# underdoc-wang/MPGCN

Measured on NVIDIA H100. Metric: OD-cells/sec (B*T*N^2), MPGCN hot path fwd+bwd, higher is better.
Workload: dtype f16

## Files before the change

mpgcn_b200/csrc/common.cuh:

```cuda
#pragma once

#include <cuda.h>
#include <cuda_fp16.h>
#include <cuda_runtime.h>
#include <stdint.h>
#include <stdio.h>

#if defined(__CUDA_ARCH__) && !defined(__CUDA_ARCH_FEAT_SM90_ALL)
#error "mpgcn_b200 must be compiled for sm_90a (-gencode arch=compute_90a,code=sm_90a)"
#endif

namespace mpgcn {

void set_error(const char* fmt, ...);
#define MPGCN_CHECK(cond, ...)                                                     \
  do {                                                                             \
    if (!(cond)) {                                                                 \
      ::mpgcn::set_error(__VA_ARGS__);                                             \
      return 1;                                                                    \
    }                                                                              \
  } while (0)
#define MPGCN_CUDA(call)                                                           \
  do {                                                                             \
    cudaError_t e__ = (call);                                                      \
// ... 7 lines not shown

#ifdef __CUDACC__
__device__ __forceinline__ uint32_t smem_u32(const void* p) {
  return static_cast<uint32_t>(__cvta_generic_to_shared(p));
}

__device__ __forceinline__ void mbar_init(uint64_t* bar, uint32_t count) {
  asm volatile("mbarrier.init.shared::cta.b64 [%0], %1;" ::"r"(smem_u32(bar)), "r"(count) : "memory");
}
__device__ __forceinline__ void fence_barrier_init() {
  asm volatile("fence.mbarrier_init.release.cluster;" ::: "memory");
}
__device__ __forceinline__ void fence_proxy_async_smem() {
  asm volatile("fence.proxy.async.shared::cta;" ::: "memory");
}
__device__ __forceinline__ void mbar_arrive_expect_tx(uint64_t* bar, uint32_t bytes) {
  asm volatile("mbarrier.arrive.expect_tx.shared::cta.b64 _, [%0], %1;" ::"r"(smem_u32(bar)), "r"(bytes) : "memory");
}
__device__ __forceinline__ void mbar_arrive(uint64_t* bar) {
  asm volatile("mbarrier.arrive.shared::cta.b64 _, [%0];" ::"r"(smem_u32(bar)) : "memory");
}
__device__ __forceinline__ bool mbar_try_wait(uint64_t* bar, uint32_t parity) {
  uint32_t ok;
  asm volatile(
      "{\n\t.reg .pred p;\n\t"
      "mbarrier.try_wait.parity.shared::cta.b64 p, [%1], %2;\n\t"
      "selp.u32 %0, 1, 0, p;\n\t}"
      : "=r"(ok)
      : "r"(smem_u32(bar)), "r"(parity)
      : "memory");
  return ok != 0;
}
static __device__ __noinline__ void mbar_wait_slow(uint64_t* bar, uint32_t parity) {
  const long long t0 = clock64();
  uint32_t spins = 0;
  while (!mbar_try_wait(bar, parity)) {
    if (((++spins) & 0xFFFu) == 0 && (clock64() - t0) > 6000000000LL) {
      printf("mpgcn_b200: mbarrier wait timed out (block %d thread %d)\n", blockIdx.x, threadIdx.x);
      __trap();
    }
  }
}
__device__ __forceinline__ void mbar_wait(uint64_t* bar, uint32_t parity) {
  if (mbar_try_wait(bar, parity)) return;
  mbar_wait_slow(bar, parity);
}
__device__ __forceinline__ void mbar_wait_inline(uint64_t* bar, uint32_t parity) {
  if (mbar_try_wait(bar, parity)) return;
  const long long t0 = clock64();
  while (!mbar_try_wait(bar, parity))
    if (clock64() - t0 > 6000000000LL) __trap();
}

__device__ __forceinline__ void tma_prefetch_desc(const CUtensorMap* map) {
  asm volatile("prefetch.tensormap [%0];" ::"l"(map) : "memory");
}
__device__ __forceinline__ void tma_load_4d(void* smem_dst, const CUtensorMap* map, uint64_t* bar,
                                            int c0, int c1, int c2, int c3) {
  asm volatile(
      "cp.async.bulk.tensor.4d.shared::cluster.global.mbarrier::complete_tx::bytes"
      " [%0], [%1, {%3, %4, %5, %6}], [%2];"
      ::"r"(smem_u32(smem_dst)), "l"(map), "r"(smem_u32(bar)), "r"(c0), "r"(c1), "r"(c2), "r"(c3)
      : "memory");
}

__device__ __forceinline__ void wgmma_fence() { asm volatile("wgmma.fence.sync.aligned;" ::: "memory"); }
__device__ __forceinline__ void wgmma_commit() { asm volatile("wgmma.commit_group.sync.aligned;" ::: "memory"); }
template <int N>
__device__ __forceinline__ void wgmma_wait() { asm volatile("wgmma.wait_group.sync.aligned %0;" ::"n"(N) : "memory"); }
__device__ __forceinline__ void named_bar_sync(int id, int count) { asm volatile("bar.sync %0, %1;" ::"r"(id), "r"(count) : "memory"); }

constexpr uint32_t GMMA_SW128 = 1u, GMMA_SW64 = 2u;
__device__ __forceinline__ uint64_t gmma_desc_hi(uint32_t sbo_bytes, uint32_t swizzle) {
  return (static_cast<uint64_t>((sbo_bytes >> 4) & 0x3FFFu) | (static_cast<uint64_t>(swizzle) << 30)) << 32;
}
__device__ __forceinline__ uint64_t gmma_desc(uint64_t hi, uint32_t smem_addr, uint32_t lbo_bytes) {
  return hi | static_cast<uint64_t>((smem_addr >> 4) & 0x3FFFu) | (static_cast<uint64_t>((lbo_bytes >> 4) & 0x3FFFu) << 16);
}

__device__ __forceinline__ void mma_16816(float (&d)[4], const uint32_t (&a)[4], uint32_t b0, uint32_t b1) {
  asm volatile("mma.sync.aligned.m16n8k16.row.col.f32.f16.f16.f32 {%0, %1, %2, %3}, {%4, %5, %6, %7}, {%8, %9}, {%0, %1, %2, %3};"
               : "+f"(d[0]), "+f"(d[1]), "+f"(d[2]), "+f"(d[3])
               : "r"(a[0]), "r"(a[1]), "r"(a[2]), "r"(a[3]), "r"(b0), "r"(b1));
}
__device__ __forceinline__ void ldmatrix_x4(uint32_t addr, uint32_t& r0, uint32_t& r1, uint32_t& r2, uint32_t& r3) {
  asm volatile("ldmatrix.sync.aligned.m8n8.x4.shared.b16 {%0, %1, %2, %3}, [%4];" : "=r"(r0), "=r"(r1), "=r"(r2), "=r"(r3) : "r"(addr));
}
__device__ __forceinline__ void ldmatrix_x4_trans(uint32_t addr, uint32_t& r0, uint32_t& r1, uint32_t& r2, uint32_t& r3) {
  asm volatile("ldmatrix.sync.aligned.m8n8.x4.trans.shared.b16 {%0, %1, %2, %3}, [%4];" : "=r"(r0), "=r"(r1), "=r"(r2), "=r"(r3) : "r"(addr));
}

__device__ __forceinline__ __half f2h_sat(float x) { return __float2half_rn(fabsf(x) > 65504.f ? copysignf(65504.f, x) : x); }
__device__ __forceinline__ uint32_t f2h2_sat_bits(float a, float b) {
  uint32_t r;
  asm("cvt.rn.satfinite.f16x2.f32 %0, %1, %2;" : "=r"(r) : "f"(b), "f"(a));
  return r;
}
#endif

enum TmapSwizzle { TMAP_SW64 = 0, TMAP_SW128 = 1 };
int make_tmap_f16(CUtensorMap* out, const void* gptr, int rank, const uint64_t* dims, const uint64_t* strides_bytes,
                  const uint32_t* box, TmapSwizzle swz);

int device_sm_count();

struct DynSmemAttr { int bytes[64]; };
int ensure_dyn_smem_impl(const void* kernel, int bytes, DynSmemAttr& cache);
template <class Kernel>
inline int ensure_dyn_smem(Kernel kernel, int bytes, DynSmemAttr& cache) {
  return ensure_dyn_smem_impl(reinterpret_cast<const void*>(kernel), bytes, cache);
}

enum ProfTag {
  PROF_FWD_A = 0, PROF_FWD_MIX, PROF_FWD_B, PROF_BWD_V, PROF_BWD_DW, PROF_BWD_MIX, PROF_BWD_DX,
  PROF_SIMT_GEMM, PROF_ELEMENTWISE, PROF_LSTM_FWD, PROF_LSTM_BWD,
  PROF_LAYER_FWD, PROF_LAYER_BWD, PROF_HEAD,
  PROF_EXCHANGE,
  PROF_NUM_TAGS
};
constexpr int PROF_FIRST_REGION_TAG = PROF_LAYER_FWD;
void prof_set_next(int tag, double flops);
void prof_take_next(int* tag, double* flops);
void prof_count(int tag);
void prof_begin(int tag, double flops, cudaStream_t s);
void prof_end(cudaStream_t s);
struct ProfRegion {
  void* a = nullptr;
  int tag;
  cudaStream_t s;
  ProfRegion(int tag, double flops, cudaStream_t s);
  ~ProfRegion();
};

}
```

mpgcn_b200/csrc/lstm_tc.cu:

```cuda
#include "kernels.h"

namespace mpgcn {
namespace lstm_tc {

template <int CH>
struct Dims {
  static constexpr int CG = CH == 1 ? 8 : CH == 3 ? 4 : 3;
  static constexpr int CELLS = 16 * CG;
  static constexpr int H = 32 * CH;
  static constexpr int G4 = 4 * H;
  static constexpr int KX = H + 16;
  static constexpr int WX_LD = KX + 8;
  static constexpr int HX_LD = KX + 8;
  static constexpr int H_LD = H + 8;
  static constexpr int DA_LD = G4 + 8;
  static constexpr int NW = CG * CH;
  static constexpr int THREADS = 32 * NW;
  static constexpr int FWD_CTAS_PER_SM = CH == 1 ? 2 : 1;
  static constexpr int BWD_CTAS_PER_SM = 1;
  static constexpr int TILE_HALVES = CELLS * H * 2;
};

constexpr int WT_LD = 136;
constexpr float kLn2 = 0.69314718055994531f;
// ... 11 lines not shown
__device__ __forceinline__ uint32_t pack2(float a, float b) {
  __half2 h = __floats2half2_rn(a, b);
  return *reinterpret_cast<uint32_t*>(&h);
}
__device__ __forceinline__ uint4 pack8(const float* v) {
  return make_uint4(pack2(v[0], v[1]), pack2(v[2], v[3]), pack2(v[4], v[5]), pack2(v[6], v[7]));
}
__device__ __forceinline__ void unpack8(const uint4& v, float* f) {
  const __half2* h2 = reinterpret_cast<const __half2*>(&v);
#pragma unroll
  for (int e = 0; e < 4; ++e) {
    const float2 t = __half22float2(h2[e]);
    f[2 * e] = t.x;
    f[2 * e + 1] = t.y;
  }
}

template <int CH>
__device__ __forceinline__ int gate_row(int r) { return (r & 127) / 32 * (32 * CH) + 32 * (r >> 7) + (r & 31); }
__device__ __forceinline__ float row_scale(int r) { return ((r & 127) >> 5) == 2 ? -2.8853900817779268f : -1.4426950408889634f; }

template <int CH>
__device__ void load_wx(__half* sWx, const float* w_ih, const float* w_hh, const float* b_ih, const float* b_hh) {
  using D = Dims<CH>;
  constexpr int NCH = D::KX / 8;
  for (int e = threadIdx.x; e < D::G4 * NCH; e += blockDim.x) {
    const int r = e / NCH, ch = e % NCH, j = gate_row<CH>(r);
    const float sc = row_scale(r);
    float v[8] = {0.f, 0.f, 0.f, 0.f, 0.f, 0.f, 0.f, 0.f};
    if (ch < D::H / 8) {
#pragma unroll
      for (int i = 0; i < 8; ++i) v[i] = sc * w_hh[(size_t)j * D::H + ch * 8 + i];
    } else if (ch == D::H / 8) {
      const float wi = sc * w_ih[j], bb = sc * (b_ih[j] + b_hh[j]);
      const float wi_hi = __half2float(__float2half_rn(wi)), b_hi = __half2float(__float2half_rn(bb));
      v[0] = wi_hi; v[1] = b_hi; v[2] = wi_hi; v[3] = wi - wi_hi; v[4] = bb - b_hi;
    }
    *reinterpret_cast<uint4*>(sWx + r * D::WX_LD + ch * 8) = pack8(v);
  }
}

__device__ __forceinline__ uint32_t x_cols(float x, int q) {
  const float x_hi = x_split_hi(x);
  return q == 0 ? pack2(x_hi, 1.f) : q == 1 ? pack2(x_split_lo(x, x_hi), x_hi) : q == 2 ? pack2(1.f, 0.f) : 0u;
}

template <int CH, class AH>
__device__ __forceinline__ void gate_mma(float (&acc)[16][4], AH&& a_h, const uint32_t (&xw)[2], uint32_t wx_addr) {
  using D = Dims<CH>;
  const int lane = threadIdx.x & 31, mi = lane >> 3;
#pragma unroll
  for (int nt = 0; nt < 16; ++nt) acc[nt][0] = acc[nt][1] = acc[nt][2] = acc[nt][3] = 0.f;
#pragma unroll
  for (int kb = 0; kb <= 2 * CH; ++kb) {
    uint32_t a[4];
    if (kb < 2 * CH) a_h(kb, a);
    else { a[0] = xw[0]; a[1] = xw[1]; a[2] = 0u; a[3] = 0u; }
#pragma unroll
    for (int pr = 0; pr < 8; ++pr) {
      uint32_t b0, b1, b2, b3;
      ldmatrix_x4(wx_addr + (uint32_t)(((16 * pr + 8 * (mi >> 1) + (lane & 7)) * D::WX_LD + 16 * kb + 8 * (mi & 1)) * 2), b0, b1, b2, b3);
      mma_16816(acc[2 * pr], a, b0, b1);
      mma_16816(acc[2 * pr + 1], a, b2, b3);
    }
  }
}

__device__ __forceinline__ void cell_update(const float (&acc)[16][4], float (&c)[2][8], float (&hv)[2][8]) {
#pragma unroll
  for (int h = 0; h < 2; ++h) {
#pragma unroll
    for (int s = 0; s < 8; ++s) {
      const int jn = s >> 1, k = 2 * h + (s & 1);
      const float ai = 1.f + ex2_(fminf(acc[jn][k], 40.f));
      const float af = 1.f + ex2_(fminf(acc[4 + jn][k], 40.f));
      const float ag = 1.f + ex2_(fminf(acc[8 + jn][k], 40.f));
      const float p = 1.f + ex2_(fminf(acc[12 + jn][k], 40.f));
      const float pig = ai * ag;
      const float r = rcp_(pig * af);
      const float gi = r * (ag * af);
      const float gg = fmaf(r + r, ai * af, -1.f);
      const float gf = r * pig;
      c[h][s] = fmaf(gf, c[h][s], gi * gg);
      const float ac = 1.f + ex2_(fminf(-2.8853900817779268f * c[h][s], 40.f));
      const float r2 = rcp_(p * ac);
      hv[h][s] = (r2 * ac) * fmaf(r2 + r2, p, -1.f);
    }
  }
}

template <int CH>
__device__ __forceinline__ float cell_grad(const float (&acc)[16][4], int h, const uint4& vc, const uint4& vcp, const float (&dh)[8],
                                           float (&dc)[8], const float* s_wih, int js, int q, float (&d)[4][8]) {
  constexpr int H = Dims<CH>::H;
  float fc[8], fcp[8];
  unpack8(vc, fc);
  unpack8(vcp, fcp);
  float dx = 0.f;
#pragma unroll
  for (int s = 0; s < 8; ++s) {
    const int jn = s >> 1, k = 2 * h + (s & 1);
    const float ai = 1.f + ex2_(fminf(acc[jn][k], 40.f));
    const float af = 1.f + ex2_(fminf(acc[4 + jn][k], 40.f));
    const float ag = 1.f + ex2_(fminf(acc[8 + jn][k], 40.f));
    const float ao = 1.f + ex2_(fminf(acc[12 + jn][k], 40.f));
    const float ac = 1.f + ex2_(fminf(-2.8853900817779268f * fc[s], 40.f));
    const float pig = ai * ag;
    const float r1 = rcp_(pig * af), r2 = rcp_(ao * ac);
    const float gi = r1 * (ag * af), gg = fmaf(r1 + r1, ai * af, -1.f), gf = r1 * pig;
    const float go = r2 * ac, tcv = fmaf(r2 + r2, ao, -1.f);
    const float dhv = dh[s];
    const float dcv = fmaf(dhv * go, fmaf(-tcv, tcv, 1.f), dc[s]);
    d[3][s] = (dhv * tcv) * fmaf(-go, go, go);
    d[0][s] = (dcv * gg) * fmaf(-gi, gi, gi);
    d[1][s] = (dcv * fcp[s]) * fmaf(-gf, gf, gf);
    d[2][s] = (dcv * gi) * fmaf(-gg, gg, 1.f);
    dc[s] = dcv * gf;
    const int u = 32 * js + 8 * jn + 2 * q + (s & 1);
    dx += d[0][s] * s_wih[u] + d[1][s] * s_wih[H + u] + d[2][s] * s_wih[2 * H + u] + d[3][s] * s_wih[3 * H + u];
  }
  return dx;
}

template <int CH>
__device__ __forceinline__ size_t save_off(long long tile, int T, int t, int warp, int kind, int lane) {
  return ((size_t)tile * T + t) * Dims<CH>::TILE_HALVES + (size_t)warp * 1024 + (size_t)kind * 512 + (size_t)lane * 16;
}

template <bool SAVE>
__global__ void __launch_bounds__(Dims<1>::THREADS, Dims<1>::FWD_CTAS_PER_SM)
lstm_fwd_tc_kernel(const float* __restrict__ x_seq, const float* __restrict__ w_ih, const float* __restrict__ w_hh,
                   const float* __restrict__ b_ih, const float* __restrict__ b_hh, float* __restrict__ hT, __half* __restrict__ saved,
                   long long cells, int T, long long NN) {
  using D = Dims<1>;
  __shared__ __align__(16) __half sWx[D::G4 * D::WX_LD];
  load_wx<1>(sWx, w_ih, w_hh, b_ih, b_hh);
  __syncthreads();
  const int warp = threadIdx.x >> 5, lane = threadIdx.x & 31, g = lane >> 2, q = lane & 3;
  const uint32_t wx_addr = smem_u32(sWx);
  const long long tiles = (cells + D::CELLS - 1) / D::CELLS;
  for (long long tile = blockIdx.x; tile < tiles; tile += gridDim.x) {
    long long cell[2];
    bool live[2];
    size_t xb[2];
    float xv[2];
#pragma unroll
    for (int h = 0; h < 2; ++h) {
      cell[h] = tile * D::CELLS + warp * 16 + g + 8 * h;
      live[h] = cell[h] < cells;
      xb[h] = live[h] ? x_base(cell[h], T, NN) : 0;
      xv[h] = live[h] ? x_seq[xb[h]] : 0.f;
    }
    float c[2][8], hv[2][8];
#pragma unroll
    for (int h = 0; h < 2; ++h)
#pragma unroll
      for (int s = 0; s < 8; ++s) { c[h][s] = 0.f; hv[h][s] = 0.f; }
    for (int t = 0; t < T; ++t) {
      uint32_t hw[8], xw[2];
#pragma unroll
      for (int h = 0; h < 2; ++h) {
#pragma unroll
        for (int jn = 0; jn < 4; ++jn) hw[4 * h + jn] = pack2(hv[h][2 * jn], hv[h][2 * jn + 1]);
        xw[h] = x_cols(xv[h], q);
      }
      float acc[16][4];
      gate_mma<1>(acc, [&](int kb, uint32_t (&a)[4]) {
        a[0] = hw[2 * kb]; a[1] = hw[4 + 2 * kb]; a[2] = hw[2 * kb + 1]; a[3] = hw[4 + 2 * kb + 1];
      }, xw, wx_addr);
#pragma unroll
      for (int h = 0; h < 2; ++h) xv[h] = (live[h] && t + 1 < T) ? x_seq[xb[h] + (size_t)(t + 1) * NN] : 0.f;
      cell_update(acc, c, hv);
      if (SAVE) {
        uint4* dc = reinterpret_cast<uint4*>(saved + save_off<1>(tile, T, t, warp, 0, lane));
        uint4* dh = reinterpret_cast<uint4*>(saved + save_off<1>(tile, T, t, warp, 1, lane));
        dc[0] = pack8(c[0]); dc[1] = pack8(c[1]);
        dh[0] = pack8(hv[0]); dh[1] = pack8(hv[1]);
      }
    }
    if (hT != nullptr) {
#pragma unroll
      for (int h = 0; h < 2; ++h)
        if (live[h]) {
#pragma unroll
          for (int jn = 0; jn < 4; ++jn)
            *reinterpret_cast<float2*>(hT + (size_t)cell[h] * D::H + 8 * jn + 2 * q) = make_float2(hv[h][2 * jn], hv[h][2 * jn + 1]);
        }
    }
  }
}

constexpr size_t kBwdSavedSmem = (size_t)(Dims<1>::G4 * Dims<1>::WX_LD + Dims<1>::H * WT_LD + 2 * Dims<1>::CELLS * Dims<1>::DA_LD +
                                          2 * Dims<1>::CELLS * Dims<1>::HX_LD) * sizeof(__half) + Dims<1>::G4 * sizeof(float);

__global__ void __launch_bounds__(Dims<1>::THREADS, Dims<1>::BWD_CTAS_PER_SM)
lstm_bwd_saved_tc_kernel(const float* __restrict__ x_seq, const float* __restrict__ w_ih, const float* __restrict__ w_hh,
                         const float* __restrict__ b_ih, const float* __restrict__ b_hh, const float* __restrict__ d_hT,
                         float* __restrict__ d_w_ih, float* __restrict__ d_w_hh, float* __restrict__ d_b, float* __restrict__ d_x,
                         const __half* __restrict__ saved, const float* __restrict__ scale2, long long cells, int T, long long NN) {
  using D = Dims<1>;
  constexpr int C = D::H, CELLS = D::CELLS;
  extern __shared__ __align__(16) uint8_t smem_raw[];
  __half* sWx = reinterpret_cast<__half*>(smem_raw);
  __half* sWT = sWx + D::G4 * D::WX_LD;
  __half* sDA = sWT + C * WT_LD;
  __half* sHX = sDA + 2 * CELLS * D::DA_LD;
  float* s_wih = reinterpret_cast<float*>(sHX + 2 * CELLS * D::HX_LD);

  load_wx<1>(sWx, w_ih, w_hh, b_ih, b_hh);
  for (int e = threadIdx.x; e < D::G4 * C; e += blockDim.x) {
    const int j = e / C, u = e % C;
    sWT[u * WT_LD + j] = __float2half_rn(w_hh[e]);
  }
  for (int j = threadIdx.x; j < D::G4; j += blockDim.x) s_wih[j] = w_ih[j];
  for (int e = threadIdx.x; e < 2 * CELLS; e += blockDim.x)
    *reinterpret_cast<uint4*>(sHX + e * D::HX_LD + 40) = make_uint4(0u, 0u, 0u, 0u);
  __syncthreads();

  const int warp = threadIdx.x >> 5, lane = threadIdx.x & 31, g = lane >> 2, q = lane & 3, mi = lane >> 3;
  const uint32_t wx_addr = smem_u32(sWx), wt_addr = smem_u32(sWT), da_addr = smem_u32(sDA), hx_addr = smem_u32(sHX);
  const long long tiles = (cells + CELLS - 1) / CELLS;
  const float S = scale2[0], invS = scale2[1];
  float dw[6][4];
#pragma unroll
  for (int nt = 0; nt < 6; ++nt) dw[nt][0] = dw[nt][1] = dw[nt][2] = dw[nt][3] = 0.f;
  int step = 0;

  for (long long tile = blockIdx.x; tile < tiles; tile += gridDim.x) {
    long long cell[2];
    bool live[2];
    size_t xb[2];
    float dh[2][8], dc[2][8];
#pragma unroll
    for (int h = 0; h < 2; ++h) {
      cell[h] = tile * CELLS + warp * 16 + g + 8 * h;
      live[h] = cell[h] < cells;
      xb[h] = live[h] ? x_base(cell[h], T, NN) : 0;
#pragma unroll
      for (int s = 0; s < 8; ++s) {
        dh[h][s] = live[h] ? d_hT[(size_t)cell[h] * C + 8 * (s >> 1) + 2 * q + (s & 1)] * S : 0.f;
        dc[h][s] = 0.f;
      }
    }
    for (int t = T - 1; t >= 0; --t, ++step) {
      uint4 vc[2], vcp[2], vhp[2];
      {
        const uint4* pc = reinterpret_cast<const uint4*>(saved + save_off<1>(tile, T, t, warp, 0, lane));
        vc[0] = pc[0]; vc[1] = pc[1];
        if (t > 0) {
          const uint4* pcp = reinterpret_cast<const uint4*>(saved + save_off<1>(tile, T, t - 1, warp, 0, lane));
          const uint4* php = reinterpret_cast<const uint4*>(saved + save_off<1>(tile, T, t - 1, warp, 1, lane));
          vcp[0] = pcp[0]; vcp[1] = pcp[1]; vhp[0] = php[0]; vhp[1] = php[1];
        } else {
          vcp[0] = vcp[1] = vhp[0] = vhp[1] = make_uint4(0u, 0u, 0u, 0u);
        }
      }
      const uint32_t hw[8] = {vhp[0].x, vhp[0].y, vhp[0].z, vhp[0].w, vhp[1].x, vhp[1].y, vhp[1].z, vhp[1].w};
      float xt[2];
      uint32_t xw[2];
#pragma unroll
      for (int h = 0; h < 2; ++h) {
        xt[h] = live[h] ? x_seq[xb[h] + (size_t)t * NN] : 0.f;
        xw[h] = x_cols(xt[h], q);
      }
      float acc[16][4];
      gate_mma<1>(acc, [&](int kb, uint32_t (&a)[4]) {
        a[0] = hw[2 * kb]; a[1] = hw[4 + 2 * kb]; a[2] = hw[2 * kb + 1]; a[3] = hw[4 + 2 * kb + 1];
      }, xw, wx_addr);

      uint32_t da[16][2];
      float dx[2];
#pragma unroll
      for (int h = 0; h < 2; ++h) {
        float d[4][8];
        dx[h] = cell_grad<1>(acc, h, vc[h], vcp[h], dh[h], dc[h], s_wih, 0, q, d);
#pragma unroll
        for (int jn = 0; jn < 4; ++jn)
#pragma unroll
          for (int gt = 0; gt < 4; ++gt) da[4 * gt + jn][h] = pack2(d[gt][2 * jn], d[gt][2 * jn + 1]);
      }
      if (d_x != nullptr) {
#pragma unroll
        for (int h = 0; h < 2; ++h) {
          float v = dx[h];
          v += __shfl_xor_sync(0xffffffffu, v, 1);
          v += __shfl_xor_sync(0xffffffffu, v, 2);
          if (q == 0 && live[h]) d_x[xb[h] + (size_t)t * NN] = v * invS;
        }
      }
      if (t > 0) {
        float adh[4][4];
#pragma unroll
        for (int nt = 0; nt < 4; ++nt) adh[nt][0] = adh[nt][1] = adh[nt][2] = adh[nt][3] = 0.f;
#pragma unroll
        for (int kb = 0; kb < 8; ++kb) {
          const uint32_t a[4] = {da[2 * kb][0], da[2 * kb][1], da[2 * kb + 1][0], da[2 * kb + 1][1]};
#pragma unroll
          for (int pr = 0; pr < 2; ++pr) {
            uint32_t b0, b1, b2, b3;
            ldmatrix_x4(wt_addr + (uint32_t)(((16 * pr + 8 * (mi >> 1) + (lane & 7)) * WT_LD + 16 * kb + 8 * (mi & 1)) * 2), b0, b1, b2, b3);
            mma_16816(adh[2 * pr], a, b0, b1);
            mma_16816(adh[2 * pr + 1], a, b2, b3);
          }
        }
#pragma unroll
        for (int h = 0; h < 2; ++h)
#pragma unroll
          for (int s = 0; s < 8; ++s) dh[h][s] = adh[s >> 1][2 * h + (s & 1)];
      }
      const int buf = step & 1;
      __half* sda = sDA + buf * CELLS * D::DA_LD;
      __half* shx = sHX + buf * CELLS * D::HX_LD;
#pragma unroll
      for (int h = 0; h < 2; ++h) {
        const int row = warp * 16 + g + 8 * h;
#pragma unroll
        for (int nt = 0; nt < 16; ++nt) *reinterpret_cast<uint32_t*>(sda + row * D::DA_LD + 8 * nt + 2 * q) = da[nt][h];
#pragma unroll
        for (int jn = 0; jn < 4; ++jn) *reinterpret_cast<uint32_t*>(shx + row * D::HX_LD + 8 * jn + 2 * q) = hw[4 * h + jn];
        *reinterpret_cast<uint32_t*>(shx + row * D::HX_LD + 32 + 2 * q) = xw[h];
      }
      __syncthreads();
      const uint32_t da_b = da_addr + (uint32_t)(buf * CELLS * D::DA_LD * 2), hx_b = hx_addr + (uint32_t)(buf * CELLS * D::HX_LD * 2);
#pragma unroll
      for (int kc = 0; kc < 8; ++kc) {
        uint32_t a[4];
        ldmatrix_x4_trans(da_b + (uint32_t)(((16 * kc + 8 * (mi >> 1) + (lane & 7)) * D::DA_LD + 16 * warp + 8 * (mi & 1)) * 2), a[0], a[1], a[2], a[3]);
#pragma unroll
        for (int pr = 0; pr < 3; ++pr) {
          uint32_t b0, b1, b2, b3;
          ldmatrix_x4_trans(hx_b + (uint32_t)(((16 * kc + 8 * (mi & 1) + (lane & 7)) * D::HX_LD + 16 * pr + 8 * (mi >> 1)) * 2), b0, b1, b2, b3);
          mma_16816(dw[2 * pr], a, b0, b1);
          mma_16816(dw[2 * pr + 1], a, b2, b3);
        }
      }
    }
  }
#pragma unroll
  for (int nt = 0; nt < 5; ++nt)
#pragma unroll
    for (int i = 0; i < 4; ++i) {
      const int j = 16 * warp + g + 8 * (i >> 1), col = 8 * nt + 2 * q + (i & 1);
      const float v = dw[nt][i] * invS;
      if (col < C) atomicAdd(&d_w_hh[j * C + col], v);
      else if (col == 32 || col == 34) atomicAdd(&d_w_ih[j], v);
      else if (col == 33) atomicAdd(&d_b[j], v);
    }
}


template <int CH>
constexpr size_t kFwdWideSmem = (size_t)(Dims<CH>::G4 * Dims<CH>::WX_LD + 2 * Dims<CH>::CELLS * Dims<CH>::H_LD) * sizeof(__half);

template <int CH, bool SAVE>
__global__ void __launch_bounds__(Dims<CH>::THREADS, Dims<CH>::FWD_CTAS_PER_SM)
lstm_fwd_tcw_kernel(const float* __restrict__ x_seq, const float* __restrict__ w_ih, const float* __restrict__ w_hh,
                    const float* __restrict__ b_ih, const float* __restrict__ b_hh, float* __restrict__ hT, __half* __restrict__ saved,
                    long long cells, int T, long long NN) {
  using D = Dims<CH>;
  constexpr int CELLS = D::CELLS;
  extern __shared__ __align__(16) uint8_t smem_raw[];
  __half* sWx = reinterpret_cast<__half*>(smem_raw);
  __half* sH = sWx + D::G4 * D::WX_LD;
  load_wx<CH>(sWx, w_ih, w_hh, b_ih, b_hh);
  __syncthreads();
  const int warp = threadIdx.x >> 5, lane = threadIdx.x & 31, g = lane >> 2, q = lane & 3;
  const int cg = warp / CH, js = warp % CH;
  const uint32_t wx_addr = smem_u32(sWx + js * 128 * D::WX_LD);
  const uint32_t h_addr = smem_u32(sH + (cg * 16 + (lane & 15)) * D::H_LD + 8 * (lane >> 4));
  const long long tiles = (cells + CELLS - 1) / CELLS;
  for (long long tile = blockIdx.x; tile < tiles; tile += gridDim.x) {
    long long cell[2];
    bool live[2];
    size_t xb[2];
    float xv[2];
#pragma unroll
    for (int h = 0; h < 2; ++h) {
      cell[h] = tile * CELLS + cg * 16 + g + 8 * h;
      live[h] = cell[h] < cells;
      xb[h] = live[h] ? x_base(cell[h], T, NN) : 0;
      xv[h] = live[h] ? x_seq[xb[h]] : 0.f;
    }
    float c[2][8];
#pragma unroll
    for (int h = 0; h < 2; ++h)
#pragma unroll
      for (int s = 0; s < 8; ++s) c[h][s] = 0.f;
    for (int t = 0; t < T; ++t) {
      uint32_t xw[2];
#pragma unroll
// ... 62 lines not shown
  const uint32_t da_addr = smem_u32(sDA + (cg * 16 + (lane & 15)) * D::DA_LD + 8 * (lane >> 4));
  const long long tiles = (cells + CELLS - 1) / CELLS;
  const float S = scale2[0], invS = scale2[1];

  for (long long tile = blockIdx.x; tile < tiles; tile += gridDim.x) {
    long long cell[2];
    bool live[2];
    size_t xb[2];
    float dh[2][8], dc[2][8];
#pragma unroll
    for (int h = 0; h < 2; ++h) {
      cell[h] = tile * CELLS + cg * 16 + g + 8 * h;
      live[h] = cell[h] < cells;
      xb[h] = live[h] ? x_base(cell[h], T, NN) : 0;
#pragma unroll
      for (int s = 0; s < 8; ++s) {
        dh[h][s] = live[h] ? d_hT[(size_t)cell[h] * D::H + 32 * js + 8 * (s >> 1) + 2 * q + (s & 1)] * S : 0.f;
        dc[h][s] = 0.f;
      }
    }
    const long long dx_cell = tile * CELLS + cg * 16 + (lane & 15);
    const bool dx_live = d_x != nullptr && js == 0 && lane < 16 && dx_cell < cells;
    const size_t dx_base = dx_live ? x_base(dx_cell, T, NN) : 0;

    for (int t = T - 1; t >= 0; --t) {
      uint32_t xw[2];
#pragma unroll
      for (int h = 0; h < 2; ++h) xw[h] = x_cols(live[h] ? x_seq[xb[h] + (size_t)t * NN] : 0.f, q);
      const __half* hp = saved + (t > 0 ? save_off<CH>(tile, T, t - 1, cg * CH, 1, lane) : 0);
      float acc[16][4];
      gate_mma<CH>(acc, [&](int kb, uint32_t (&a)[4]) {
        if (t == 0) { a[0] = a[1] = a[2] = a[3] = 0u; return; }
        const uint2* p = reinterpret_cast<const uint2*>(hp + (kb >> 1) * 1024);
        const uint2 r0 = __ldg(p + (kb & 1)), r1 = __ldg(p + 2 + (kb & 1));
        a[0] = r0.x; a[1] = r1.x; a[2] = r0.y; a[3] = r1.y;
      }, xw, wx_addr);

      uint4 vc[2], vcp[2];
      {
        const uint4* pc = reinterpret_cast<const uint4*>(saved + save_off<CH>(tile, T, t, warp, 0, lane));
        vc[0] = pc[0]; vc[1] = pc[1];
        if (t > 0) {
          const uint4* pcp = reinterpret_cast<const uint4*>(saved + save_off<CH>(tile, T, t - 1, warp, 0, lane));
          vcp[0] = pcp[0]; vcp[1] = pcp[1];
        } else {
          vcp[0] = vcp[1] = make_uint4(0u, 0u, 0u, 0u);
        }
      }
      uint32_t da[16][2];
      float dx[2];
#pragma unroll
      for (int h = 0; h < 2; ++h) {
        float d[4][8];
        dx[h] = cell_grad<CH>(acc, h, vc[h], vcp[h], dh[h], dc[h], s_wih, js, q, d);
#pragma unroll
        for (int jn = 0; jn < 4; ++jn)
#pragma unroll
          for (int gt = 0; gt < 4; ++gt) {
            const float inv_s = gt == 2 ? -0.5f * kLn2 : -kLn2;
            da[4 * gt + jn][h] = pack2(inv_s * d[gt][2 * jn], inv_s * d[gt][2 * jn + 1]);
          }
        dx[h] += __shfl_xor_sync(0xffffffffu, dx[h], 1);
        dx[h] += __shfl_xor_sync(0xffffffffu, dx[h], 2);
      }
      named_bar_sync(1 + cg, 32 * CH);
#pragma unroll
      for (int h = 0; h < 2; ++h) {
        const int row = cg * 16 + g + 8 * h;
#pragma unroll
        for (int nt = 0; nt < 16; ++nt) *reinterpret_cast<uint32_t*>(sDA + row * D::DA_LD + 128 * js + 8 * nt + 2 * q) = da[nt][h];
        if (q == 0) sDX[row * CH + js] = dx[h];
      }
      named_bar_sync(1 + cg, 32 * CH);
      if (dx_live) {
        float v = 0.f;
#pragma unroll
        for (int sl = 0; sl < CH; ++sl) v += sDX[(cg * 16 + lane) * CH + sl];
        d_x[dx_base + (size_t)t * NN] = v * invS;
      }
      {
        __half* rec = da_rec + (((size_t)tile * T + t) * CELLS + cg * 16) * D::G4 + 128 * js;
#pragma unroll
        for (int i = 0; i < 8; ++i) {
          const int idx = 32 * i + lane, row = idx >> 4, ch = idx & 15;
          *reinterpret_cast<uint4*>(rec + (size_t)row * D::G4 + 8 * ch) =
              *reinterpret_cast<const uint4*>(sDA + (cg * 16 + row) * D::DA_LD + 128 * js + 8 * ch);
        }
      }
      if (t > 0) {
        float adh[4][4];
#pragma unroll
        for (int nt = 0; nt < 4; ++nt) adh[nt][0] = adh[nt][1] = adh[nt][2] = adh[nt][3] = 0.f;
#pragma unroll 4
        for (int kb = 0; kb < D::G4 / 16; ++kb) {
          uint32_t a[4];
          ldmatrix_x4(da_addr + 32 * kb, a[0], a[1], a[2], a[3]);
#pragma unroll
          for (int pr = 0; pr < 2; ++pr) {
            uint32_t b0, b1, b2, b3;
            ldmatrix_x4_trans(wx_all + (uint32_t)(((16 * kb + 8 * (mi & 1) + (lane & 7)) * D::WX_LD + 32 * js + 16 * pr + 8 * (mi >> 1)) * 2),
                              b0, b1, b2, b3);
            mma_16816(adh[2 * pr], a, b0, b1);
            mma_16816(adh[2 * pr + 1], a, b2, b3);
          }
        }
#pragma unroll
        for (int h = 0; h < 2; ++h)
// ... 90 lines not shown
using lstm_tc::Dims;

bool lstm_tc_supported(int T, int C) { return (C == 32 || C == 96 || C == 128) && T >= 1 && T <= 256; }

template <int CH>
static int lstm_grid(long long cells, int ctas_per_sm) {
  const long long tiles = (cells + Dims<CH>::CELLS - 1) / Dims<CH>::CELLS;
  long long g = (long long)ctas_per_sm * device_sm_count();
  return (int)(g < tiles ? g : tiles);
}

static long long lstm_tc_padded_cells(int B, long long NN, int C) {
  const long long tc = C == 32 ? Dims<1>::CELLS : C == 96 ? Dims<3>::CELLS : Dims<4>::CELLS;
  return ((long long)B * NN + tc - 1) / tc * tc;
}

size_t lstm_tc_saved_bytes(int B, int T, long long NN, int C) {
  return (size_t)lstm_tc_padded_cells(B, NN, C) * T * 2 * C * sizeof(__half);
}

static size_t lstm_tcw_da_bytes(int B, int T, long long NN, int C) {
  return (size_t)lstm_tc_padded_cells(B, NN, C) * T * 4 * C * sizeof(__half);
}

static size_t lstm_tc_bwd_saved_workspace_bytes(int B, int T, long long NN, int C) {
  return 1024 + (C == 32 ? 0 : align_up(lstm_tcw_da_bytes(B, T, NN, C), 256));
}

size_t lstm_tc_bwd_workspace_bytes(int B, int T, long long NN, int C) {
  return lstm_tc_bwd_saved_workspace_bytes(B, T, NN, C) + align_up(lstm_tc_saved_bytes(B, T, NN, C), 256);
}

template <int CH>
static int lstm_forward_tcw(const float* x_seq, const float* w_ih, const float* w_hh, const float* b_ih, const float* b_hh, float* hT,
                            void* saved, long long cells, int T, long long NN, cudaStream_t st) {
  using D = Dims<CH>;
  auto kern = saved ? lstm_tc::lstm_fwd_tcw_kernel<CH, true> : lstm_tc::lstm_fwd_tcw_kernel<CH, false>;
  constexpr size_t smem = lstm_tc::kFwdWideSmem<CH>;
  static DynSmemAttr attr_t = {}, attr_f = {};
  if (int e = ensure_dyn_smem(kern, (int)smem, saved ? attr_t : attr_f)) return e;
  prof_begin(PROF_LSTM_FWD, 8.0 * D::H * (D::H + 1) * (double)cells * T, st);
  kern<<<lstm_grid<CH>(cells, D::FWD_CTAS_PER_SM), D::THREADS, smem, st>>>(x_seq, w_ih, w_hh, b_ih, b_hh, hT,
                                                                           static_cast<__half*>(saved), cells, T, NN);
  prof_end(st);
  MPGCN_CUDA(cudaGetLastError());
  return 0;
}

static int lstm_backward_h32(const float* x_seq, const float* w_ih, const float* w_hh, const float* b_ih, const float* b_hh,
                             const float* d_hT, float* d_w_ih, float* d_w_hh, float* d_b, float* d_x, const void* saved,
                             void* , const float* scale2, long long cells, int T, long long NN, cudaStream_t st) {
  using D = Dims<1>;
  if (d_x) MPGCN_CUDA(cudaMemsetAsync(d_x, 0, sizeof(float) * (size_t)cells * T, st));
  static DynSmemAttr attr_b = {};
  if (int e = ensure_dyn_smem(lstm_tc::lstm_bwd_saved_tc_kernel, (int)lstm_tc::kBwdSavedSmem, attr_b)) return e;
  prof_begin(PROF_LSTM_BWD, 12.0 * D::H * (D::H + 1) * (double)cells * T, st);
  lstm_tc::lstm_bwd_saved_tc_kernel<<<lstm_grid<1>(cells, D::BWD_CTAS_PER_SM), D::THREADS, lstm_tc::kBwdSavedSmem, st>>>(
      x_seq, w_ih, w_hh, b_ih, b_hh, d_hT, d_w_ih, d_w_hh, d_b, d_x, static_cast<const __half*>(saved), scale2, cells, T, NN);
  prof_end(st);
  MPGCN_CUDA(cudaGetLastError());
  return 0;
}

template <int CH>
static int lstm_backward_tcw(const float* x_seq, const float* w_ih, const float* w_hh, const float* b_ih, const float* b_hh,
                             const float* d_hT, float* d_w_ih, float* d_w_hh, float* d_b, float* d_x, const void* saved, void* da_rec,
                             const float* scale2, long long cells, int T, long long NN, cudaStream_t st) {
  using D = Dims<CH>;
  constexpr size_t smem = lstm_tc::kWalkSmem<CH>;
  static DynSmemAttr attr_b = {};
  if (int e = ensure_dyn_smem(lstm_tc::lstm_bwd_walk_tcw_kernel<CH>, (int)smem, attr_b)) return e;
  prof_begin(PROF_LSTM_BWD, 8.0 * D::H * (D::H + 1) * (double)cells * T, st);
  lstm_tc::lstm_bwd_walk_tcw_kernel<CH><<<lstm_grid<CH>(cells, D::BWD_CTAS_PER_SM), D::THREADS, smem, st>>>(
      x_seq, w_ih, w_hh, b_ih, b_hh, d_hT, d_x, static_cast<const __half*>(saved), static_cast<__half*>(da_rec), scale2, cells, T, NN);
  prof_end(st);
  MPGCN_CUDA(cudaGetLastError());
  const long long records = (cells + D::CELLS - 1) / D::CELLS * T;
  long long splits = 4LL * device_sm_count() / CH;
  if (splits > records) splits = records;
  prof_begin(PROF_LSTM_BWD, 4.0 * D::H * (D::H + 1) * (double)cells * T, st);
  lstm_tc::lstm_dw_tcw_kernel<CH><<<dim3(CH, (unsigned)splits), lstm_tc::DW_THREADS, 0, st>>>(
      x_seq, static_cast<const __half*>(saved), static_cast<const __half*>(da_rec), d_w_ih, d_w_hh, d_b, scale2, cells, T, NN);
  prof_end(st);
  MPGCN_CUDA(cudaGetLastError());
  return 0;
}

int lstm_last_forward_tc(const float* x_seq, const float* w_ih, const float* w_hh, const float* b_ih, const float* b_hh, float* hT,
                         void* saved, int B, int T, long long NN, int C, cudaStream_t st) {
  using D = Dims<1>;
  const long long cells = (long long)B * NN;
  MPGCN_CHECK(saved == nullptr || (reinterpret_cast<uintptr_t>(saved) & 15) == 0, "lstm forward: saved buffer must be 16-byte aligned");
  if (C == 96) return lstm_forward_tcw<3>(x_seq, w_ih, w_hh, b_ih, b_hh, hT, saved, cells, T, NN, st);
  if (C == 128) return lstm_forward_tcw<4>(x_seq, w_ih, w_hh, b_ih, b_hh, hT, saved, cells, T, NN, st);
  MPGCN_CHECK(C == D::H, "lstm forward: no tensor-core kernel for hidden=%d", C);
  auto kern = saved ? lstm_tc::lstm_fwd_tc_kernel<true> : lstm_tc::lstm_fwd_tc_kernel<false>;
  prof_begin(PROF_LSTM_FWD, 8.0 * C * (C + 1) * (double)cells * T, st);
  kern<<<lstm_grid<1>(cells, D::FWD_CTAS_PER_SM), D::THREADS, 0, st>>>(x_seq, w_ih, w_hh, b_ih, b_hh, hT, static_cast<__half*>(saved),
                                                                       cells, T, NN);
  prof_end(st);
  MPGCN_CUDA(cudaGetLastError());
  return 0;
}

int lstm_last_backward_tc(const float* x_seq, const float* w_ih, const float* w_hh, const float* b_ih, const float* b_hh,
                          const float* d_hT, float* d_w_ih, float* d_w_hh, float* d_b_ih, float* d_b_hh, float* d_x, const void* saved,
                          int B, int T, long long NN, int C, void* ws, size_t ws_bytes, const float* d_hT_absmax, cudaStream_t st) {
  const long long cells = (long long)B * NN;
  const size_t need = saved ? lstm_tc_bwd_saved_workspace_bytes(B, T, NN, C) : lstm_tc_bwd_workspace_bytes(B, T, NN, C);
  MPGCN_CHECK(ws != nullptr && ws_bytes >= need, "lstm backward: workspace too small (%zu < %zu)", ws_bytes, need);
// ... 26 lines not shown
```

Before: 487.8 million.

## Pipeline LSTM backward with cp.async ring and mbarrier-decoupled weight-gradient GEMM

The saved-state LSTM backward kernel now prefetches the saved c/h states and x inputs through a 3-slot cp.async ring in shared memory. The block-wide __syncthreads before the weight-gradient MMA is replaced by full/empty mbarriers, so each warp computes the dW product for the previous step while the next step proceeds. The kernel is templated on whether d_x is needed so the dx arithmetic can be compiled out. The x-column bias MMA uses a smaller m16n8k8 and the dW accumulator tile shrinks from 6 to 5 n-tiles. This costs more shared memory, which may lower occupancy, and adds barrier and ring-slot bookkeeping.

```diff
diff --git a/mpgcn_b200/csrc/common.cuh b/mpgcn_b200/csrc/common.cuh
--- a/mpgcn_b200/csrc/common.cuh
+++ b/mpgcn_b200/csrc/common.cuh
@@ -83,6 +83,16 @@
     if (clock64() - t0 > 6000000000LL) __trap();
 }
 
+__device__ __forceinline__ void cp_async16(void* smem_dst, const void* src) {
+  asm volatile("cp.async.cg.shared.global [%0], [%1], 16;" ::"r"(smem_u32(smem_dst)), "l"(src) : "memory");
+}
+__device__ __forceinline__ void cp_async4(void* smem_dst, const void* src) {
+  asm volatile("cp.async.ca.shared.global [%0], [%1], 4;" ::"r"(smem_u32(smem_dst)), "l"(src) : "memory");
+}
+__device__ __forceinline__ void cp_async_commit() { asm volatile("cp.async.commit_group;" ::: "memory"); }
+template <int N>
+__device__ __forceinline__ void cp_async_wait() { asm volatile("cp.async.wait_group %0;" ::"n"(N) : "memory"); }
+
 __device__ __forceinline__ void tma_prefetch_desc(const CUtensorMap* map) {
   asm volatile("prefetch.tensormap [%0];" ::"l"(map) : "memory");
 }
@@ -113,6 +123,17 @@
   asm volatile("mma.sync.aligned.m16n8k16.row.col.f32.f16.f16.f32 {%0, %1, %2, %3}, {%4, %5, %6, %7}, {%8, %9}, {%0, %1, %2, %3};"
                : "+f"(d[0]), "+f"(d[1]), "+f"(d[2]), "+f"(d[3])
                : "r"(a[0]), "r"(a[1]), "r"(a[2]), "r"(a[3]), "r"(b0), "r"(b1));
+}
+__device__ __forceinline__ void mma_1688(float (&d)[4], uint32_t a0, uint32_t a1, uint32_t b0) {
+  asm volatile("mma.sync.aligned.m16n8k8.row.col.f32.f16.f16.f32 {%0, %1, %2, %3}, {%4, %5}, {%6}, {%0, %1, %2, %3};"
+               : "+f"(d[0]), "+f"(d[1]), "+f"(d[2]), "+f"(d[3])
+               : "r"(a0), "r"(a1), "r"(b0));
+}
+__device__ __forceinline__ void ldmatrix_x2(uint32_t addr, uint32_t& r0, uint32_t& r1) {
+  asm volatile("ldmatrix.sync.aligned.m8n8.x2.shared.b16 {%0, %1}, [%2];" : "=r"(r0), "=r"(r1) : "r"(addr));
+}
+__device__ __forceinline__ void ldmatrix_x2_trans(uint32_t addr, uint32_t& r0, uint32_t& r1) {
+  asm volatile("ldmatrix.sync.aligned.m8n8.x2.trans.shared.b16 {%0, %1}, [%2];" : "=r"(r0), "=r"(r1) : "r"(addr));
 }
 __device__ __forceinline__ void ldmatrix_x4(uint32_t addr, uint32_t& r0, uint32_t& r1, uint32_t& r2, uint32_t& r3) {
   asm volatile("ldmatrix.sync.aligned.m8n8.x4.shared.b16 {%0, %1, %2, %3}, [%4];" : "=r"(r0), "=r"(r1), "=r"(r2), "=r"(r3) : "r"(addr));
diff --git a/mpgcn_b200/csrc/lstm_tc.cu b/mpgcn_b200/csrc/lstm_tc.cu
--- a/mpgcn_b200/csrc/lstm_tc.cu
+++ b/mpgcn_b200/csrc/lstm_tc.cu
@@ -87,10 +87,9 @@
 #pragma unroll
   for (int nt = 0; nt < 16; ++nt) acc[nt][0] = acc[nt][1] = acc[nt][2] = acc[nt][3] = 0.f;
 #pragma unroll
-  for (int kb = 0; kb <= 2 * CH; ++kb) {
+  for (int kb = 0; kb < 2 * CH; ++kb) {
     uint32_t a[4];
-    if (kb < 2 * CH) a_h(kb, a);
-    else { a[0] = xw[0]; a[1] = xw[1]; a[2] = 0u; a[3] = 0u; }
+    a_h(kb, a);
 #pragma unroll
     for (int pr = 0; pr < 8; ++pr) {
       uint32_t b0, b1, b2, b3;
@@ -98,6 +97,13 @@
       mma_16816(acc[2 * pr], a, b0, b1);
       mma_16816(acc[2 * pr + 1], a, b2, b3);
     }
+  }
+#pragma unroll
+  for (int pr = 0; pr < 8; ++pr) {
+    uint32_t b0, b1;
+    ldmatrix_x2(wx_addr + (uint32_t)(((16 * pr + 8 * (mi & 1) + (lane & 7)) * D::WX_LD + 32 * CH) * 2), b0, b1);
+    mma_1688(acc[2 * pr], xw[0], xw[1], b0);
+    mma_1688(acc[2 * pr + 1], xw[0], xw[1], b1);
   }
 }
 
@@ -124,7 +130,7 @@
   }
 }
 
-template <int CH>
+template <int CH, bool DX>
 __device__ __forceinline__ float cell_grad(const float (&acc)[16][4], int h, const uint4& vc, const uint4& vcp, const float (&dh)[8],
                                            float (&dc)[8], const float* s_wih, int js, int q, float (&d)[4][8]) {
   constexpr int H = Dims<CH>::H;
@@ -151,8 +157,10 @@
     d[1][s] = (dcv * fcp[s]) * fmaf(-gf, gf, gf);
     d[2][s] = (dcv * gi) * fmaf(-gg, gg, 1.f);
     dc[s] = dcv * gf;
-    const int u = 32 * js + 8 * jn + 2 * q + (s & 1);
-    dx += d[0][s] * s_wih[u] + d[1][s] * s_wih[H + u] + d[2][s] * s_wih[2 * H + u] + d[3][s] * s_wih[3 * H + u];
+    if (DX) {
+      const int u = 32 * js + 8 * jn + 2 * q + (s & 1);
+      dx += d[0][s] * s_wih[u] + d[1][s] * s_wih[H + u] + d[2][s] * s_wih[2 * H + u] + d[3][s] * s_wih[3 * H + u];
+    }
   }
   return dx;
 }
@@ -225,9 +233,14 @@
   }
 }
 
-constexpr size_t kBwdSavedSmem = (size_t)(Dims<1>::G4 * Dims<1>::WX_LD + Dims<1>::H * WT_LD + 2 * Dims<1>::CELLS * Dims<1>::DA_LD +
-                                          2 * Dims<1>::CELLS * Dims<1>::HX_LD) * sizeof(__half) + Dims<1>::G4 * sizeof(float);
-
+constexpr int kBwdRing = 3;
+constexpr size_t kBwdSavedSmem =
+    (size_t)(Dims<1>::G4 * Dims<1>::WX_LD + Dims<1>::H * WT_LD + kBwdRing * Dims<1>::CELLS * (Dims<1>::DA_LD + Dims<1>::HX_LD)) * sizeof(__half) +
+    (size_t)kBwdRing * Dims<1>::NW * 2048 +
+    (size_t)kBwdRing * Dims<1>::THREADS * 2 * sizeof(float) +
+    Dims<1>::G4 * sizeof(float) + 2 * kBwdRing * sizeof(uint64_t);
+
+template <bool DX>
 __global__ void __launch_bounds__(Dims<1>::THREADS, Dims<1>::BWD_CTAS_PER_SM)
 lstm_bwd_saved_tc_kernel(const float* __restrict__ x_seq, const float* __restrict__ w_ih, const float* __restrict__ w_hh,
                          const float* __restrict__ b_ih, const float* __restrict__ b_hh, const float* __restrict__ d_hT,
@@ -239,8 +252,12 @@
   __half* sWx = reinterpret_cast<__half*>(smem_raw);
   __half* sWT = sWx + D::G4 * D::WX_LD;
   __half* sDA = sWT + C * WT_LD;
-  __half* sHX = sDA + 2 * CELLS * D::DA_LD;
-  float* s_wih = reinterpret_cast<float*>(sHX + 2 * CELLS * D::HX_LD);
+  __half* sHX = sDA + kBwdRing * CELLS * D::DA_LD;
+  uint4* sST = reinterpret_cast<uint4*>(sHX + kBwdRing * CELLS * D::HX_LD);
+  float* sX = reinterpret_cast<float*>(sST + kBwdRing * D::NW * 128);
+  float* s_wih = sX + kBwdRing * D::THREADS * 2;
+  uint64_t* full = reinterpret_cast<uint64_t*>(s_wih + D::G4);
+  uint64_t* empty = full + kBwdRing;
 
   load_wx<1>(sWx, w_ih, w_hh, b_ih, b_hh);
   for (int e = threadIdx.x; e < D::G4 * C; e += blockDim.x) {
@@ -248,18 +265,69 @@
     sWT[u * WT_LD + j] = __float2half_rn(w_hh[e]);
   }
   for (int j = threadIdx.x; j < D::G4; j += blockDim.x) s_wih[j] = w_ih[j];
-  for (int e = threadIdx.x; e < 2 * CELLS; e += blockDim.x)
-    *reinterpret_cast<uint4*>(sHX + e * D::HX_LD + 40) = make_uint4(0u, 0u, 0u, 0u);
+  if (threadIdx.x == 0)
+    for (int s = 0; s < kBwdRing; ++s) { mbar_init(&full[s], D::NW); mbar_init(&empty[s], D::NW); }
   __syncthreads();
 
   const int warp = threadIdx.x >> 5, lane = threadIdx.x & 31, g = lane >> 2, q = lane & 3, mi = lane >> 3;
   const uint32_t wx_addr = smem_u32(sWx), wt_addr = smem_u32(sWT), da_addr = smem_u32(sDA), hx_addr = smem_u32(sHX);
   const long long tiles = (cells + CELLS - 1) / CELLS;
   const float S = scale2[0], invS = scale2[1];
-  float dw[6][4];
-#pragma unroll
-  for (int nt = 0; nt < 6; ++nt) dw[nt][0] = dw[nt][1] = dw[nt][2] = dw[nt][3] = 0.f;
-  int step = 0;
+  float dw[5][4];
+#pragma unroll
+  for (int nt = 0; nt < 5; ++nt) dw[nt][0] = dw[nt][1] = dw[nt][2] = dw[nt][3] = 0.f;
+
+  long long pf_tile = blockIdx.x;
+  int pf_t = T - 1;
+  size_t pf_xb[2];
+  auto pf_cells = [&]() {
+#pragma unroll
+    for (int h = 0; h < 2; ++h) {
+      const long long cell = pf_tile * CELLS + warp * 16 + g + 8 * h;
+      pf_xb[h] = pf_tile < tiles && cell < cells ? x_base(cell, T, NN) : ~(size_t)0;
+    }
+  };
+  auto fetch = [&](int slot) {
+    if (pf_tile < tiles) {
+      const uint4* pc = reinterpret_cast<const uint4*>(saved + save_off<1>(pf_tile, T, pf_t, warp, 0, lane));
+      const uint4* ph = reinterpret_cast<const uint4*>(saved + save_off<1>(pf_tile, T, pf_t, warp, 1, lane));
+      uint4* dst = sST + (slot * D::NW + warp) * 128 + lane;
+      cp_async16(dst, pc); cp_async16(dst + 32, pc + 1); cp_async16(dst + 64, ph); cp_async16(dst + 96, ph + 1);
+#pragma unroll
+      for (int h = 0; h < 2; ++h)
+        if (pf_xb[h] != ~(size_t)0) cp_async4(sX + (slot * D::THREADS + threadIdx.x) * 2 + h, x_seq + pf_xb[h] + (size_t)pf_t * NN);
+    }
+    cp_async_commit();
+    if (--pf_t < 0) { pf_t = T - 1; pf_tile += gridDim.x; pf_cells(); }
+  };
+  auto dwext = [&](int slot, uint32_t phase) {
+    mbar_wait_inline(&full[slot], phase);
+    const uint32_t da_b = da_addr + (uint32_t)(slot * CELLS * D::DA_LD * 2), hx_b = hx_addr + (uint32_t)(slot * CELLS * D::HX_LD * 2);
+#pragma unroll
+    for (int kc = 0; kc < 8; ++kc) {
+      uint32_t a[4];
+      ldmatrix_x4_trans(da_b + (uint32_t)(((16 * kc + 8 * (mi >> 1) + (lane & 7)) * D::DA_LD + 16 * warp + 8 * (mi & 1)) * 2), a[0], a[1], a[2], a[3]);
+#pragma unroll
+      for (int pr = 0; pr < 2; ++pr) {
+        uint32_t b0, b1, b2, b3;
+        ldmatrix_x4_trans(hx_b + (uint32_t)(((16 * kc + 8 * (mi & 1) + (lane & 7)) * D::HX_LD + 16 * pr + 8 * (mi >> 1)) * 2), b0, b1, b2, b3);
+        mma_16816(dw[2 * pr], a, b0, b1);
+        mma_16816(dw[2 * pr + 1], a, b2, b3);
+      }
+      uint32_t b0, b1;
+      ldmatrix_x2_trans(hx_b + (uint32_t)(((16 * kc + 8 * (mi & 1) + (lane & 7)) * D::HX_LD + 32) * 2), b0, b1);
+      mma_16816(dw[4], a, b0, b1);
+    }
+    __syncwarp();
+    if (lane == 0) mbar_arrive(&empty[slot]);
+  };
+
+  pf_cells();
+  fetch(0);
+  fetch(1);
+  int slot = 0, prev_slot = 0;
+  uint32_t phase = 0, prev_phase = 0;
+  bool have_prev = false;
 
   for (long long tile = blockIdx.x; tile < tiles; tile += gridDim.x) {
     long long cell[2];
@@ -270,34 +338,30 @@
     for (int h = 0; h < 2; ++h) {
       cell[h] = tile * CELLS + warp * 16 + g + 8 * h;
       live[h] = cell[h] < cells;
-      xb[h] = live[h] ? x_base(cell[h], T, NN) : 0;
+      xb[h] = DX && live[h] ? x_base(cell[h], T, NN) : 0;
 #pragma unroll
       for (int s = 0; s < 8; ++s) {
         dh[h][s] = live[h] ? d_hT[(size_t)cell[h] * C + 8 * (s >> 1) + 2 * q + (s & 1)] * S : 0.f;
         dc[h][s] = 0.f;
       }
     }
-    for (int t = T - 1; t >= 0; --t, ++step) {
-      uint4 vc[2], vcp[2], vhp[2];
-      {
-        const uint4* pc = reinterpret_cast<const uint4*>(saved + save_off<1>(tile, T, t, warp, 0, lane));
-        vc[0] = pc[0]; vc[1] = pc[1];
-        if (t > 0) {
-          const uint4* pcp = reinterpret_cast<const uint4*>(saved + save_off<1>(tile, T, t - 1, warp, 0, lane));
-          const uint4* php = reinterpret_cast<const uint4*>(saved + save_off<1>(tile, T, t - 1, warp, 1, lane));
-          vcp[0] = pcp[0]; vcp[1] = pcp[1]; vhp[0] = php[0]; vhp[1] = php[1];
-        } else {
-          vcp[0] = vcp[1] = vhp[0] = vhp[1] = make_uint4(0u, 0u, 0u, 0u);
-        }
+    uint4 vc[2];
+    for (int t = T - 1; t >= 0; --t) {
+      fetch(slot == 0 ? kBwdRing - 1 : slot - 1);
+      cp_async_wait<1>();
+      const uint4* st0 = sST + (slot * D::NW + warp) * 128 + lane;
+      const uint4* st1 = sST + ((slot + 1 == kBwdRing ? 0 : slot + 1) * D::NW + warp) * 128 + lane;
+      if (t == T - 1) { vc[0] = st0[0]; vc[1] = st0[32]; }
+      uint4 vcp[2], vhp[2];
+      if (t > 0) {
+        vcp[0] = st1[0]; vcp[1] = st1[32]; vhp[0] = st1[64]; vhp[1] = st1[96];
+      } else {
+        vcp[0] = vcp[1] = vhp[0] = vhp[1] = make_uint4(0u, 0u, 0u, 0u);
       }
       const uint32_t hw[8] = {vhp[0].x, vhp[0].y, vhp[0].z, vhp[0].w, vhp[1].x, vhp[1].y, vhp[1].z, vhp[1].w};
-      float xt[2];
       uint32_t xw[2];
 #pragma unroll
-      for (int h = 0; h < 2; ++h) {
-        xt[h] = live[h] ? x_seq[xb[h] + (size_t)t * NN] : 0.f;
-        xw[h] = x_cols(xt[h], q);
-      }
+      for (int h = 0; h < 2; ++h) xw[h] = x_cols(live[h] ? sX[(slot * D::THREADS + threadIdx.x) * 2 + h] : 0.f, q);
       float acc[16][4];
       gate_mma<1>(acc, [&](int kb, uint32_t (&a)[4]) {
         a[0] = hw[2 * kb]; a[1] = hw[4 + 2 * kb]; a[2] = hw[2 * kb + 1]; a[3] = hw[4 + 2 * kb + 1];
@@ -308,13 +372,13 @@
 #pragma unroll
       for (int h = 0; h < 2; ++h) {
         float d[4][8];
-        dx[h] = cell_grad<1>(acc, h, vc[h], vcp[h], dh[h], dc[h], s_wih, 0, q, d);
+        dx[h] = cell_grad<1, DX>(acc, h, vc[h], vcp[h], dh[h], dc[h], s_wih, 0, q, d);
 #pragma unroll
         for (int jn = 0; jn < 4; ++jn)
 #pragma unroll
           for (int gt = 0; gt < 4; ++gt) da[4 * gt + jn][h] = pack2(d[gt][2 * jn], d[gt][2 * jn + 1]);
       }
-      if (d_x != nullptr) {
+      if (DX) {
 #pragma unroll
         for (int h = 0; h < 2; ++h) {
           float v = dx[h];
@@ -343,9 +407,9 @@
 #pragma unroll
           for (int s = 0; s < 8; ++s) dh[h][s] = adh[s >> 1][2 * h + (s & 1)];
       }
-      const int buf = step & 1;
-      __half* sda = sDA + buf * CELLS * D::DA_LD;
-      __half* shx = sHX + buf * CELLS * D::HX_LD;
+      mbar_wait_inline(&empty[slot], phase ^ 1u);
+      __half* sda = sDA + slot * CELLS * D::DA_LD;
+      __half* shx = sHX + slot * CELLS * D::HX_LD;
 #pragma unroll
       for (int h = 0; h < 2; ++h) {
         const int row = warp * 16 + g + 8 * h;
@@ -355,22 +419,18 @@
         for (int jn = 0; jn < 4; ++jn) *reinterpret_cast<uint32_t*>(shx + row * D::HX_LD + 8 * jn + 2 * q) = hw[4 * h + jn];
         *reinterpret_cast<uint32_t*>(shx + row * D::HX_LD + 32 + 2 * q) = xw[h];
       }
-      __syncthreads();
-      const uint32_t da_b = da_addr + (uint32_t)(buf * CELLS * D::DA_LD * 2), hx_b = hx_addr + (uint32_t)(buf * CELLS * D::HX_LD * 2);
-#pragma unroll
-      for (int kc = 0; kc < 8; ++kc) {
-        uint32_t a[4];
-        ldmatrix_x4_trans(da_b + (uint32_t)(((16 * kc + 8 * (mi >> 1) + (lane & 7)) * D::DA_LD + 16 * warp + 8 * (mi & 1)) * 2), a[0], a[1], a[2], a[3]);
-#pragma unroll
-        for (int pr = 0; pr < 3; ++pr) {
-          uint32_t b0, b1, b2, b3;
-          ldmatrix_x4_trans(hx_b + (uint32_t)(((16 * kc + 8 * (mi & 1) + (lane & 7)) * D::HX_LD + 16 * pr + 8 * (mi >> 1)) * 2), b0, b1, b2, b3);
-          mma_16816(dw[2 * pr], a, b0, b1);
-          mma_16816(dw[2 * pr + 1], a, b2, b3);
-        }
-      }
-    }
-  }
+      __syncwarp();
+      if (lane == 0) mbar_arrive(&full[slot]);
+      if (have_prev) dwext(prev_slot, prev_phase);
+      have_prev = true;
+      prev_slot = slot;
+      prev_phase = phase;
+      if (++slot == kBwdRing) { slot = 0; phase ^= 1u; }
+      vc[0] = vcp[0];
+      vc[1] = vcp[1];
+    }
+  }
+  if (have_prev) dwext(prev_slot, prev_phase);
 #pragma unroll
   for (int nt = 0; nt < 5; ++nt)
 #pragma unroll
@@ -539,7 +599,7 @@
 #pragma unroll
       for (int h = 0; h < 2; ++h) {
         float d[4][8];
-        dx[h] = cell_grad<CH>(acc, h, vc[h], vcp[h], dh[h], dc[h], s_wih, js, q, d);
+        dx[h] = cell_grad<CH, true>(acc, h, vc[h], vcp[h], dh[h], dc[h], s_wih, js, q, d);
 #pragma unroll
         for (int jn = 0; jn < 4; ++jn)
 #pragma unroll
@@ -736,10 +796,11 @@
                              void* , const float* scale2, long long cells, int T, long long NN, cudaStream_t st) {
   using D = Dims<1>;
   if (d_x) MPGCN_CUDA(cudaMemsetAsync(d_x, 0, sizeof(float) * (size_t)cells * T, st));
-  static DynSmemAttr attr_b = {};
-  if (int e = ensure_dyn_smem(lstm_tc::lstm_bwd_saved_tc_kernel, (int)lstm_tc::kBwdSavedSmem, attr_b)) return e;
+  auto kern = d_x ? lstm_tc::lstm_bwd_saved_tc_kernel<true> : lstm_tc::lstm_bwd_saved_tc_kernel<false>;
+  static DynSmemAttr attr_x = {}, attr_n = {};
+  if (int e = ensure_dyn_smem(kern, (int)lstm_tc::kBwdSavedSmem, d_x ? attr_x : attr_n)) return e;
   prof_begin(PROF_LSTM_BWD, 12.0 * D::H * (D::H + 1) * (double)cells * T, st);
-  lstm_tc::lstm_bwd_saved_tc_kernel<<<lstm_grid<1>(cells, D::BWD_CTAS_PER_SM), D::THREADS, lstm_tc::kBwdSavedSmem, st>>>(
+  kern<<<lstm_grid<1>(cells, D::BWD_CTAS_PER_SM), D::THREADS, lstm_tc::kBwdSavedSmem, st>>>(
       x_seq, w_ih, w_hh, b_ih, b_hh, d_hT, d_w_ih, d_w_hh, d_b, d_x, static_cast<const __half*>(saved), scale2, cells, T, NN);
   prof_end(st);
   MPGCN_CUDA(cudaGetLastError());
```

After: 505.0 million, median of 6. 1.04x the previous value.
